# Wuziyi616/multi_part_assembly

Measured on AMD Instinct MI355X. Metric: train-step parts/sec (BxP) at N=1000 pts, higher is better.
Workload: dtype f32

## Files before the change

### multi_part_assembly_amd/csrc/coop_reduce.h

```cpp
#pragma once

#include <hip/hip_runtime.h>

namespace mpa {

template <int U, typename Load, typename Use>
__device__ __forceinline__ void batched_rows(int g, int G, int rows, Load load, Use use) {
  using T = decltype(load(0));
  int i = g;
  for (; i + (U - 1) * G < rows; i += U * G) {
    T t[U];
#pragma unroll
    for (int u = 0; u < U; ++u) t[u] = load(i + u * G);
#pragma unroll
    for (int u = 0; u < U; ++u) use(i + u * G, t[u]);
  }
  for (; i < rows; i += G) use(i, load(i));
}


constexpr int kSlices = 16;

constexpr int kEB = 64;

__device__ __forceinline__ void coop_store(double* p, double v) {
  __hip_atomic_store(reinterpret_cast<unsigned long long*>(p), (unsigned long long)__double_as_longlong(v), __ATOMIC_RELAXED,
                     __HIP_MEMORY_SCOPE_AGENT);
}
__device__ __forceinline__ double coop_load(const double* p) {
  return __longlong_as_double((long long)__hip_atomic_load(reinterpret_cast<const unsigned long long*>(p), __ATOMIC_RELAXED,
                                                           __HIP_MEMORY_SCOPE_AGENT));
}

struct CoopWs {
  double* stage;
  unsigned* ticket;
};

template <typename Row>
__device__ __forceinline__ bool coop_colsum(int total, int C, int c, const CoopWs ws, Row row, double& s0,
                                            double& s1) {
  __shared__ double sm[kSlices][64][2];
  __shared__ bool last;
  const int cl = threadIdx.x & 63, slice = threadIdx.x >> 6;
  const int g = blockIdx.y, G = gridDim.y;
  constexpr int U = kEB / kSlices;
  double x[U], y[U];
  bool ok[U];
#pragma unroll
  for (int u = 0; u < U; ++u) {
    const int e = g * kEB + slice + u * kSlices;
    row(e < total ? e : total - 1, ok[u], x[u], y[u]);
    ok[u] = ok[u] && e < total;
  }
  double a = 0.0, b = 0.0;
#pragma unroll
  for (int u = 0; u < U; ++u) {
    if (ok[u]) {
      a += x[u];
      b += y[u];
    }
  }
  sm[slice][cl][0] = a;
  sm[slice][cl][1] = b;
  __syncthreads();
  if (slice == 0) {
    a = b = 0.0;
#pragma unroll
    for (int k = 0; k < kSlices; ++k) {
      a += sm[k][cl][0];
      b += sm[k][cl][1];
    }
    coop_store(ws.stage + ((long long)g * C + c) * 2, a);
    coop_store(ws.stage + ((long long)g * C + c) * 2 + 1, b);
    asm volatile("s_waitcnt vmcnt(0)" ::: "memory");
  }
  __syncthreads();
  if (threadIdx.x == 0) last = atomicAdd(ws.ticket + blockIdx.x, 1u) == (unsigned)(G - 1);
  __syncthreads();
  if (!last) return false;
  a = b = 0.0;
  batched_rows<4>(slice, kSlices, G,
                  [&](int gg) {
                    const double* p = ws.stage + ((long long)gg * C + c) * 2;
                    return make_double2(coop_load(p), coop_load(p + 1));
                  },
                  [&](int, const double2 t) {
                    a += t.x;
                    b += t.y;
                  });
  sm[slice][cl][0] = a;
  sm[slice][cl][1] = b;
  __syncthreads();
  s0 = s1 = 0.0;
  if (slice == 0) {
#pragma unroll
    for (int k = 0; k < kSlices; ++k) {
      s0 += sm[k][cl][0];
      s1 += sm[k][cl][1];
    }
  }
  if (threadIdx.x == 0) ws.ticket[blockIdx.x] = 0u;
  return true;
}

}
```

### multi_part_assembly_amd/csrc/pn_bwd_q.h

```cpp

#ifdef PN_TIMING
#define PN_T_DECL unsigned long long t_busy = 0, t_mark = __builtin_amdgcn_s_memtime(), t_start = t_mark;
#define PN_BAR                                         \
  {                                                    \
    t_busy += __builtin_amdgcn_s_memtime() - t_mark;   \
    __syncthreads();                                   \
    t_mark = __builtin_amdgcn_s_memtime();             \
  }
#define PN_T_REPORT(ROLE)                                                                                              \
  if (blockIdx.x == 5 && lane == 0)                                                                                    \
    printf("K=%d FIRST=%d %s wave %d: units %d busy %llu of %llu cycles\n", K, (int)FIRST, ROLE, wave, n_it, t_busy, \
           __builtin_amdgcn_s_memtime() - t_start);
#else
#define PN_T_DECL
#define PN_BAR __syncthreads();
#define PN_T_REPORT(ROLE)
#endif
#define PN_LDS __attribute__((address_space(3)))
typedef short pn_s16x4 __attribute__((ext_vector_type(4)));
typedef short pn_s16x8 __attribute__((ext_vector_type(8)));
typedef unsigned int pn_u32x4 __attribute__((ext_vector_type(4)));

__device__ __forceinline__ pn_bf16x8 pn_tr_frag(const unsigned char* p, int stride) {
  const pn_s16x4 a = __builtin_amdgcn_ds_read_tr16_b64_v4i16((PN_LDS pn_s16x4*)p);
  const pn_s16x4 b = __builtin_amdgcn_ds_read_tr16_b64_v4i16((PN_LDS pn_s16x4*)(p + 4 * stride));
  const pn_s16x8 v = {a[0], a[1], a[2], a[3], b[0], b[1], b[2], b[3]};
  return __builtin_bit_cast(pn_bf16x8, v);
}

__device__ __forceinline__ void pn_split4(const float v[4], pn_bf16x4& ph, pn_bf16x4& pm, pn_bf16x4& pl) {
#pragma unroll
  for (int u = 0; u < 4; ++u) {
    ph[u] = (__bf16)v[u];
    const float r1 = v[u] - (float)ph[u];
    pm[u] = (__bf16)r1;
    pl[u] = (__bf16)(r1 - (float)pm[u]);
  }
}

typedef float pn_f32x2 __attribute__((ext_vector_type(2)));
typedef __bf16 pn_bf16x2 __attribute__((ext_vector_type(2)));
__device__ __forceinline__ void pn_split2v(pn_f32x2 x, pn_bf16x2& h, pn_bf16x2& m, pn_bf16x2& l) {
  h = __builtin_convertvector(x, pn_bf16x2);
  const pn_f32x2 r = x - __builtin_convertvector(h, pn_f32x2);
  m = __builtin_convertvector(r, pn_bf16x2);
  const pn_f32x2 t = r - __builtin_convertvector(m, pn_f32x2);
  l = __builtin_convertvector(t, pn_bf16x2);
}
__device__ __forceinline__ void pn_split4v(pn_f32x2 a, pn_f32x2 b, pn_bf16x4& ph, pn_bf16x4& pm, pn_bf16x4& pl) {
  pn_bf16x2 h0, m0, l0, h1, m1, l1;
  pn_split2v(a, h0, m0, l0);
  pn_split2v(b, h1, m1, l1);
  ph = pn_bf16x4{h0[0], h0[1], h1[0], h1[1]};
  pm = pn_bf16x4{m0[0], m0[1], m1[0], m1[1]};
  pl = pn_bf16x4{l0[0], l0[1], l1[0], l1[1]};
}

__device__ __forceinline__ void pn_fmac(float& acc, float a, float b) {
  asm volatile("v_fmac_f32 %0, %1, %2" : "+v"(acc) : "v"(a), "v"(b));
}

#define PN_MFMA6(ACC, AH, AM, AL, BH, BM, BL)                          \
  ACC = __builtin_amdgcn_mfma_f32_32x32x16_bf16(AH, BH, ACC, 0, 0, 0); \
  ACC = __builtin_amdgcn_mfma_f32_32x32x16_bf16(AH, BM, ACC, 0, 0, 0); \
  ACC = __builtin_amdgcn_mfma_f32_32x32x16_bf16(AM, BH, ACC, 0, 0, 0); \
  ACC = __builtin_amdgcn_mfma_f32_32x32x16_bf16(AM, BM, ACC, 0, 0, 0); \
  ACC = __builtin_amdgcn_mfma_f32_32x32x16_bf16(AH, BL, ACC, 0, 0, 0); \
  ACC = __builtin_amdgcn_mfma_f32_32x32x16_bf16(AL, BH, ACC, 0, 0, 0);

__global__ void pn_bwd_q_prep_kernel(const float* __restrict__ w, const float* __restrict__ coef, int K, int CIN,
                                     float* __restrict__ q) {
  const int k = blockIdx.x, d = threadIdx.x;
  float acc = 0.0f;
  if (k < CIN) {
#pragma unroll 8
    for (int c = 0; c < K; ++c) acc = __builtin_fmaf(coef[K + c] * w[(long long)c * CIN + k], w[(long long)c * CIN + d], acc);
  } else {
#pragma unroll 8
    for (int c = 0; c < K; ++c) acc = __builtin_fmaf(coef[2 * K + c], w[(long long)c * CIN + d], acc);
  }
  q[(long long)k * CIN + d] = acc;
}

__host__ __device__ constexpr int pn_bwd_q_elems(int K, int CIN, bool first) {
  return K * CIN + CIN * CIN + CIN + (first ? 192 + 12 : 0);
}

template <int N, typename F>
__device__ __forceinline__ void pn_static_for(F&& f) {
  if constexpr (N > 0) {
    pn_static_for<N - 1>(f);
    f(std::integral_constant<int, N - 1>{});
  }
}

struct PnWTile {
  signed char a, b, kind, orow, ocol;
};
template <int K>
struct PnWPlan;
template <>
struct PnWPlan<64> {
  static constexpr int TPW = 2;
  static constexpr PnWTile t[4][2] = {{{0, 8, 0, 0, 0}, {8, 8, 1, 0, 0}},
                                      {{0, 9, 0, 0, 1}, {8, 9, 1, 0, 1}},
                                      {{1, 8, 0, 1, 0}, {-1, -1, 0, 0, 0}},
                                      {{1, 9, 0, 1, 1}, {9, 9, 1, 1, 1}}};
  static constexpr int zc[4] = {0, 0, 1, 1};
  static constexpr bool uses(int w, int code) {
    for (int i = 0; i < TPW; ++i)
      if (t[w][i].a >= 0 && (t[w][i].a == code || t[w][i].b == code)) return true;
    return false;
  }
};
template <>
struct PnWPlan<128> {
  static constexpr int TPW = 3;
  static constexpr PnWTile t[4][3] = {{{0, 8, 0, 0, 0}, {0, 9, 0, 0, 1}, {8, 8, 1, 0, 0}},
                                      {{1, 8, 0, 1, 0}, {1, 9, 0, 1, 1}, {8, 9, 1, 0, 1}},
                                      {{2, 8, 0, 2, 0}, {2, 9, 0, 2, 1}, {9, 9, 1, 1, 1}},
                                      {{3, 8, 0, 3, 0}, {3, 9, 0, 3, 1}, {-1, -1, 0, 0, 0}}};
  static constexpr int zc[4] = {0, 1, 2, 3};
  static constexpr bool uses(int w, int code) {
    for (int i = 0; i < TPW; ++i)
      if (t[w][i].a >= 0 && (t[w][i].a == code || t[w][i].b == code)) return true;
    return false;
  }
};

template <int K, int CIN, int RB, int NS, int ND, int NW, bool FIRST, int KPN = 1>
__global__ __launch_bounds__(64 * (NS + ND + NW), (NS + ND + NW + 3) / 4) void pn_bwd_q_kernel(
    const float* __restrict__ dz, const float* __restrict__ y_prev, const float* __restrict__ bn_prev,
    const float* __restrict__ w, const float* __restrict__ coef, const float* __restrict__ q,
    const int* __restrict__ vlist, int N, float* __restrict__ dz_prev, float* __restrict__ partial,
    float* __restrict__ dwpart, const float* __restrict__ wt1) {
  constexpr int SZ = 6 * K + 16, SA = 6 * CIN + 16;
  constexpr int RT = RB / 32, CT = CIN / 32;
  constexpr int KZ = K / 16, KA = CIN / 16, KW = RB / 16;
  constexpr int NTS = 64 * NS, QK = K / 4, QC = CIN / 4, RG = NTS / QC;
  constexpr int NLZ = RB * QK / NTS, NLY = RB * QC / NTS;
  constexpr int ELEMS = pn_bwd_q_elems(K, CIN, FIRST);
  constexpr int OUTP = RB * CIN;
  static_assert(ND == RT * CT * KPN && RB * QK % NTS == 0 && RB * QC % NTS == 0 && NTS % QK == 0 && NTS % QC == 0, "shapes");
  static_assert(!FIRST || CIN == 64, "the recomputed input is the 64-channel first layer");
  __shared__ __attribute__((aligned(16))) unsigned char pz[2][RB * SZ];
  __shared__ __attribute__((aligned(16))) unsigned char pa[2][RB * SA];
  __shared__ __attribute__((aligned(16))) unsigned char wl[CIN * SZ];
  __shared__ __attribute__((aligned(16))) float outp[2][KPN][OUTP];
  const int wave = __builtin_amdgcn_readfirstlane(threadIdx.x >> 6), lane = threadIdx.x & 63, j = lane & 31, hh = lane >> 5;
  const int TB = (N + RB - 1) / RB, U = vlist[0] * TB, G = gridDim.x;
  const int n_it = (int)blockIdx.x < U ? (U - (int)blockIdx.x + G - 1) / G : 0;
  auto part_of = [&](int it) {
    const int u = (int)blockIdx.x + it * G;
    return u < U && it >= 0 ? vlist[4 + u / TB] : 0;
  };
  auto n0_of = [&](int it) { return (((int)blockIdx.x + it * G) % TB) * RB; };

  for (int e = threadIdx.x; e < CIN * (K / 4); e += blockDim.x) {
    const int d = e % CIN, k4 = e / CIN;
    float v[4];
#pragma unroll
    for (int u = 0; u < 4; ++u) v[u] = coef[4 * k4 + u] * w[(long long)(4 * k4 + u) * CIN + d];
    pn_bf16x4 ph, pm, pl;
    pn_split4(v, ph, pm, pl);
    unsigned char* p = wl + d * SZ + 8 * k4;
// ... 618 lines not shown
#pragma unroll
      for (int r = 0; r < 16; ++r) o[acc_row(r, hh) * CIN] = acc[r];
      PN_BAR
    }
    PN_T_REPORT("dgrad")
  } else {
    const int ww = wave - NS - ND;
    const int g16 = lane >> 4, i16 = lane & 15;
    const int trow = 8 * (g16 >> 1) + (i16 >> 2), tcol = 16 * (g16 & 1) + 4 * (i16 & 3);
    const int offa = trow * SA + 2 * tcol;
    constexpr int TPW = PnGPlan::TPW;
    f32x16 acc[TPW];
#pragma unroll
    for (int i = 0; i < TPW; ++i) acc[i] = f32x16{0};
    __syncthreads();
    PN_T_DECL
    auto run = [&](auto w_tag) {
      constexpr int W = decltype(w_tag)::value;
      for (int it = 0; it < n_it; ++it) {
        const unsigned char* ba = pa[it & 1] + offa;
        pn_bf16x8 f[4][3];
#pragma unroll
        for (int ks = 0; ks < KW; ++ks) {
          pn_static_for<4>([&](auto c_tag) {
            constexpr int c = decltype(c_tag)::value;
            if constexpr (PnGPlan::uses(W, c)) {
#pragma unroll
              for (int pl = 0; pl < 3; ++pl) f[c][pl] = pn_tr_frag(ba + 16 * ks * SA + 2 * CIN * pl + 64 * c, SA);
            }
          });
          pn_static_for<TPW>([&](auto i_tag) {
            constexpr int i = decltype(i_tag)::value;
            constexpr PnGTile tl = PnGPlan::t[W][i];
            if constexpr (tl.a >= 0) {
              PN_MFMA6(acc[i], f[tl.a][0], f[tl.a][1], f[tl.a][2], f[tl.b][0], f[tl.b][1], f[tl.b][2])
            }
          });
        }
        PN_BAR
      }
      float* out = dwpart + (long long)blockIdx.x * ELEMS;
      pn_static_for<TPW>([&](auto i_tag) {
        constexpr int i = decltype(i_tag)::value;
        constexpr PnGTile tl = PnGPlan::t[W][i];
        if constexpr (tl.a >= 0) {
#pragma unroll
          for (int r = 0; r < 16; ++r) {
            const int ra = 32 * tl.a + acc_row(r, hh), cb = 32 * tl.b + j;
            out[ra * CIN + cb] = acc[i][r];
            if (tl.a != tl.b) out[cb * CIN + ra] = acc[i][r];
          }
        }
      });
    };
    if (ww == 0) run(std::integral_constant<int, 0>{});
    else if (ww == 1) run(std::integral_constant<int, 1>{});
    else if (ww == 2) run(std::integral_constant<int, 2>{});
    else run(std::integral_constant<int, 3>{});
    PN_T_REPORT("gram")
  }
  __syncthreads();
  {
    const float* scr = reinterpret_cast<const float*>(&pa[0][0]);
    float* out = dwpart + (long long)blockIdx.x * ELEMS;
    const int t = threadIdx.x;
    if (t < 3 * CIN) {
      const int qq = t / CIN, c = t % CIN;
      float s = 0.0f;
#pragma unroll
      for (int g = 0; g < RG; ++g) s += scr[(qq * RG + g) * CIN + c];
      if (qq == 0) out[CIN * CIN + c] = s;
      else partial[((long long)blockIdx.x * CIN + c) * 2 + (qq - 1)] = s;
    }
  }
}

struct PnFinish {
  const float* red[3];
  const float* w[3];
  const float* coef[3];
  float* dw[3];
  int K[3], CIN[3], first[4];
  const float* w1;
  const float* coef1;
  float* dw1;
  int first_layer;
};
__global__ __launch_bounds__(256) void pn_bwd_finish_kernel(const PnFinish f) {
  if ((int)blockIdx.x == f.first[3]) {
    const int t = threadIdx.x;
    if (t >= 192) return;
    const int c = t / 3, k = t % 3, i = f.first_layer;
    const float* x = f.red[i] + f.K[i] * f.CIN[i] + f.CIN[i] * f.CIN[i] + f.CIN[i];
    const float* pp = x + 192;
    float wg = 0.0f;
#pragma unroll
    for (int jx = 0; jx < 3; ++jx) {
      const int a = jx < k ? jx : k, b = jx < k ? k : jx;
      wg = __builtin_fmaf(f.w1[c * 3 + jx], pp[a == 0 ? b : (a == 1 ? 2 + b : 5)], wg);
    }
    f.dw1[t] = f.coef1[c] * x[t] + f.coef1[64 + c] * wg + f.coef1[128 + c] * pp[6 + k];
    return;
  }
  int i = 0;
#pragma unroll
  for (int qq = 1; qq < 3; ++qq) i += (int)blockIdx.x >= f.first[qq] ? 1 : 0;
  const int K = f.K[i], CIN = f.CIN[i];
  const int e = ((int)blockIdx.x - f.first[i]) * 256 + threadIdx.x;
  if (e >= K * CIN) return;
  const int c = e / CIN, d = e % CIN;
  const float* T = f.red[i];
  const float* Gm = T + K * CIN;
  const float* asum = Gm + CIN * CIN;
  const float* wr = f.w[i] + (long long)c * CIN;
  float wg = 0.0f;
#pragma unroll 8
  for (int k = 0; k < CIN; ++k) {
    const float g = (k >> 5) <= (d >> 5) ? Gm[k * CIN + d] : Gm[d * CIN + k];
    wg = __builtin_fmaf(wr[k], g, wg);
  }
  f.dw[i][e] = f.coef[i][c] * T[e] + f.coef[i][K + c] * wg + f.coef[i][2 * K + c] * asum[d];
}
```

### multi_part_assembly_amd/csrc/pointnet.hip

```cpp
#include <type_traits>

#include "common.h"
#include "coop_reduce.h"

namespace {

constexpr int kT = 256;
using mpa::CoopWs;
using mpa::coop_colsum;
using mpa::kEB;
using mpa::kSlices;

typedef float f32x16 __attribute__((ext_vector_type(16)));

__device__ __forceinline__ int acc_row(int reg, int half) { return (reg & 3) + 8 * (reg >> 2) + 4 * half; }


__global__ __launch_bounds__(1024) void pn_count_kernel(const float* __restrict__ valids, int M, int N,
                                                        float* __restrict__ count, unsigned* __restrict__ ticket,
                                                        int* __restrict__ vlist, const float* __restrict__ w1 = nullptr,
                                                        float* __restrict__ wt1 = nullptr) {
  __shared__ int wcnt[16];
  if (threadIdx.x < 4) ticket[threadIdx.x] = 0u;
  if (w1 != nullptr && threadIdx.x < 192) wt1[(threadIdx.x % 3) * 64 + threadIdx.x / 3] = w1[threadIdx.x];
// ... 3 lines not shown
    const int m = m0 + threadIdx.x;
    const bool ok = m < M && valids[m] != 0.0f;
    const unsigned long long b = __ballot(ok);
    if (lane == 0) wcnt[wave] = __popcll(b);
    __syncthreads();
    int before = 0, total = 0;
#pragma unroll
    for (int k = 0; k < 16; ++k) {
      const int c = wcnt[k];
      before += k < wave ? c : 0;
      total += c;
    }
    if (ok) vlist[4 + base + before + __popcll(b & ((1ull << lane) - 1ull))] = m;
    base += total;
    __syncthreads();
  }
  if (threadIdx.x == 0) {
    count[0] = (float)base * (float)N;
    vlist[0] = base;
  }
}

__device__ __forceinline__ bool reduce_partials(const float* __restrict__ partial,
                                                const float* __restrict__ valids, int M, int splits, int C,
                                                int c, const CoopWs ws, double& s0, double& s1) {
  return coop_colsum(M * splits, C, c, ws,
                     [&](int e, bool& ok, double& x, double& y) {
                       const float2 v = *reinterpret_cast<const float2*>(partial + ((long long)e * C + c) * 2);
                       ok = valids == nullptr || valids[e / splits] != 0.0f;
                       x = (double)v.x;
                       y = (double)v.y;
                     },
                     s0, s1);
}

__global__ __launch_bounds__(64 * kSlices) void pn_bn_finalize_kernel(
    const float* __restrict__ partial, const float* __restrict__ valids, int M, int splits, int C,
    const float* __restrict__ count, const float* __restrict__ gamma, const float* __restrict__ beta,
    float* __restrict__ running_mean, float* __restrict__ running_var, float momentum, float eps,
    float* __restrict__ bn, const CoopWs cw) {
  const int c = blockIdx.x * 64 + (threadIdx.x & 63);
  double s, ss;
  if (!reduce_partials(partial, valids, M, splits, C, c, cw, s, ss)) return;
  if (threadIdx.x >= 64) return;
  const double n = (double)count[0];
  if (n == 0.0) {
    bn[c] = 0.0f;
    bn[C + c] = beta[c];
    bn[2 * C + c] = 0.0f;
    bn[3 * C + c] = 0.0f;
    return;
  }
  const double mean = s / n;
  double var = ss / n - mean * mean;
  if (var < 0.0) var = 0.0;
  const float invstd = (float)(1.0 / __builtin_sqrt(var + (double)eps));
  const float scale = gamma[c] * invstd;
  bn[c] = scale;
  bn[C + c] = beta[c] - (float)mean * scale;
  bn[2 * C + c] = (float)mean;
  bn[3 * C + c] = invstd;
  if (running_mean != nullptr) {
    const double unbiased = n > 1.0 ? var * n / (n - 1.0) : var;
    running_mean[c] = (1.0f - momentum) * running_mean[c] + momentum * (float)mean;
    running_var[c] = (1.0f - momentum) * running_var[c] + momentum * (float)unbiased;
  }
}

__global__ void pn_bn_from_running_kernel(int C, const float* __restrict__ gamma,
                                          const float* __restrict__ beta,
                                          const float* __restrict__ running_mean,
                                          const float* __restrict__ running_var, float eps,
                                          float* __restrict__ bn) {
  const int c = blockIdx.x * 64 + threadIdx.x;
  if (c >= C) return;
  const float invstd = 1.0f / __builtin_sqrtf(running_var[c] + eps);
  const float scale = gamma[c] * invstd;
  bn[c] = scale;
  bn[C + c] = beta[c] - running_mean[c] * scale;
  bn[2 * C + c] = running_mean[c];
  bn[3 * C + c] = invstd;
}

__device__ __forceinline__ void write_coef(float* __restrict__ coef, int C, int c, float gamma,
                                           const float* __restrict__ bn, double s1, double s2, double n) {
  const float mean = bn[2 * C + c], invstd = bn[3 * C + c];
  const float alpha = gamma * invstd;
  if (n == 0.0) {
    coef[c] = coef[C + c] = coef[2 * C + c] = 0.0f;
    return;
  }
  const float gammap = (float)(-(double)alpha * s2 / n * (double)invstd);
  coef[c] = alpha;
  coef[C + c] = gammap;
  coef[2 * C + c] = (float)(-(double)alpha * s1 / n - (double)gammap * (double)mean);
}

__global__ __launch_bounds__(64 * kSlices) void pn_bwd_coef_kernel(
    const float* __restrict__ partial, const float* __restrict__ valids, int M, int splits, int C,
    const float* __restrict__ count, const float* __restrict__ gamma, const float* __restrict__ bn,
    float* __restrict__ coef, float* __restrict__ dgamma, float* __restrict__ dbeta, const CoopWs cw) {
  const int c = blockIdx.x * 64 + (threadIdx.x & 63);
  double s1, s2;
  if (!reduce_partials(partial, valids, M, splits, C, c, cw, s1, s2)) return;
  if (threadIdx.x >= 64) return;
  write_coef(coef, C, c, gamma[c], bn, s1, s2, (double)count[0]);
  dgamma[c] = (float)s2;
  dbeta[c] = (float)s1;
}

__global__ __launch_bounds__(64 * kSlices) void pn_bwd_top_kernel(
    const float* __restrict__ gfeat, const int* __restrict__ argmax, const float* __restrict__ ybest,
    const float* __restrict__ valids, int M, int F, const float* __restrict__ count,
    const float* __restrict__ gamma, const float* __restrict__ bn, float* __restrict__ coef,
    float* __restrict__ dgamma, float* __restrict__ dbeta, const CoopWs cw) {
  const int c = blockIdx.x * 64 + (threadIdx.x & 63);
  const float mean = bn[2 * F + c], invstd = bn[3 * F + c];
  double s1, s2;
  const bool last = coop_colsum(M, F, c, cw,
                                [&](int m, bool& ok, double& x, double& y) {
                                  const long long o = (long long)m * F + c;
                                  const float g = gfeat[o];
                                  ok = valids[m] != 0.0f && argmax[o] >= 0;
                                  x = (double)g;
                                  y = (double)g * (double)((ybest[o] - mean) * invstd);
                                },
                                s1, s2);
  if (!last || threadIdx.x >= 64) return;
  write_coef(coef, F, c, gamma[c], bn, s1, s2, (double)count[0]);
  dgamma[c] = (float)s2;
  dbeta[c] = (float)s1;
}

struct Top2 {
  float v1, v2;
  int n1, n2;
};
constexpr int kNoIdx = 0x7fffffff;

__device__ __forceinline__ Top2 top2_empty() { return Top2{-__builtin_inff(), -__builtin_inff(), kNoIdx, kNoIdx}; }
__device__ __forceinline__ bool top2_before(float y, int n, float y2, int n2) {
  return y > y2 || (y == y2 && n < n2);
}
__device__ __forceinline__ void top2_push(Top2& t, float y, int n) {
  const bool g1 = y > t.v1, g2 = y > t.v2;
  t.v2 = g1 ? t.v1 : (g2 ? y : t.v2);
  t.n2 = g1 ? t.n1 : (g2 ? n : t.n2);
  t.v1 = g1 ? y : t.v1;
  t.n1 = g1 ? n : t.n1;
}
__device__ __forceinline__ Top2 top2_merge(const Top2 a, const Top2 b) {
  Top2 r;
  if (top2_before(b.v1, b.n1, a.v1, a.n1)) {
    r.v1 = b.v1;
    r.n1 = b.n1;
    const bool s = top2_before(a.v1, a.n1, b.v2, b.n2);
    r.v2 = s ? a.v1 : b.v2;
    r.n2 = s ? a.n1 : b.n2;
  } else {
    r.v1 = a.v1;
    r.n1 = a.n1;
    const bool s = top2_before(a.v2, a.n2, b.v1, b.n1);
    r.v2 = s ? a.v2 : b.v1;
    r.n2 = s ? a.n2 : b.n1;
  }
  return r;
}
__device__ __forceinline__ Top2 top2_shfl_xor(const Top2 t, int mask) {
  return Top2{__shfl_xor(t.v1, mask, 64), __shfl_xor(t.v2, mask, 64), __shfl_xor(t.n1, mask, 64),
              __shfl_xor(t.n2, mask, 64)};
}

__global__ void pn_top_finalize_kernel(const float* __restrict__ topv, const int* __restrict__ topn,
                                       const float* __restrict__ bn, const float* __restrict__ valids,
                                       const float* __restrict__ y4, const float* __restrict__ bn4,
                                       const float* __restrict__ w5, int M, int N, int F, int C4, int splits,
                                       float* __restrict__ feat, int* __restrict__ argmax,
                                       float* __restrict__ ybest) {
// ... 202 lines not shown
      float yv[UB];
#pragma unroll
      for (int u = 0; u < UB; ++u) {
        const int i = slice + (u0 + u) * S, arg = arg_s[i], mm = m0 + i < M ? m0 + i : M - 1;
        yv[u] = y4[((long long)mm * N + (arg >= 0 ? arg : 0)) * C4 + ci];
      }
      __builtin_amdgcn_sched_barrier(0);
#pragma unroll
      for (int u = 0; u < UB; ++u) {
        const int i = slice + (u0 + u) * S;
        if (arg_s[i] >= 0) acc = __builtin_fmaf(g_s[i], __builtin_fmaxf(__builtin_fmaf(yv[u], sc, sh), 0.0f), acc);
      }
    }
    __syncthreads();
  }
  float wg = 0.0f;
#pragma unroll
  for (int k = 0; k < C4 / S; ++k) wg = __builtin_fmaf(wk[k], gk[k], wg);
  sm[0][slice][ci] = acc;
  sm[1][slice][ci] = wg;
  __syncthreads();
  if (slice != 0) return;
  float sparse = 0.0f;
  wg = 0.0f;
#pragma unroll
  for (int k = 0; k < S; ++k) {
    sparse += sm[0][k][ci];
    wg += sm[1][k][ci];
  }
  dw5[(long long)c * C4 + ci] = coef[c] * sparse + coef[F + c] * wg + coef[2 * F + c] * gram[C4 * C4 + ci];
}

__device__ __forceinline__ float first_layer_y(float a0, float a1, float a2, float w0, float w1, float w2) {
  float v = a0 * w0;
  v = __builtin_fmaf(a1, w1, v);
  return __builtin_fmaf(a2, w2, v);
}

template <bool STORE>
__global__ __launch_bounds__(kT) void pn_fwd_first_kernel(const float* __restrict__ pts,
                                                          const float* __restrict__ wt,
                                                          const float* __restrict__ valids, int N,
                                                          float* __restrict__ y_out,
                                                          float* __restrict__ partial) {
  __shared__ float tile[kT / 64][64][65];
  __shared__ float red[kT / 64][64][2];
  const int m = blockIdx.y;
  if (valids[m] == 0.0f) return;
  const int wave = threadIdx.x >> 6, lane = threadIdx.x & 63;
  const int n0 = blockIdx.x * kT + wave * 64, n = n0 + lane;
  const long long row = (long long)m * N + (n < N ? n : N - 1);
  const int rows_here = N - n0 < 64 ? (N - n0 < 0 ? 0 : N - n0) : 64;
  const float a0 = pts[row * 3 + 0], a1 = pts[row * 3 + 1], a2 = pts[row * 3 + 2];
#pragma unroll
  for (int c = 0; c < 64; ++c) tile[wave][lane][c] = first_layer_y(a0, a1, a2, wt[c], wt[64 + c], wt[128 + c]);
  __builtin_amdgcn_wave_barrier();
  float s = 0.0f, ss = 0.0f;
  float* dst = y_out + ((long long)m * N + n0) * 64 + lane;
  for (int i = 0; i < rows_here; ++i) {
    const float v = tile[wave][i][lane];
    if constexpr (STORE) dst[(long long)i * 64] = v;
    s += v;
    ss = __builtin_fmaf(v, v, ss);
  }
  red[wave][lane][0] = s;
  red[wave][lane][1] = ss;
  __syncthreads();
  if (threadIdx.x < 64) {
    float t0 = 0.0f, t1 = 0.0f;
#pragma unroll
    for (int w = 0; w < kT / 64; ++w) {
      t0 += red[w][threadIdx.x][0];
      t1 += red[w][threadIdx.x][1];
    }
    const long long blk = (long long)m * gridDim.x + blockIdx.x;
    partial[(blk * 64 + threadIdx.x) * 2 + 0] = t0;
    partial[(blk * 64 + threadIdx.x) * 2 + 1] = t1;
  }
}

typedef __bf16 pn_bf16x8 __attribute__((ext_vector_type(8)));
typedef __bf16 pn_bf16x4 __attribute__((ext_vector_type(4)));

__global__ __launch_bounds__(64 * kSlices) void pn_wgrad_reduce_kernel(const float* __restrict__ dwpart,
                                                                      const float* __restrict__ valids,
                                                                      int M, int elems,
                                                                      float* __restrict__ dw) {
  __shared__ float sm[kSlices][64];
  const int el = threadIdx.x & 63, slice = threadIdx.x >> 6, i = blockIdx.x * 64 + el;
  float s = 0.0f;
  if (i < elems) {
    constexpr int U = 8;
    for (int m0 = slice; m0 < M; m0 += kSlices * U) {
      float v[U], ok[U];
#pragma unroll
      for (int u = 0; u < U; ++u) {
        const int m = m0 + u * kSlices, mm = m < M ? m : M - 1;
        v[u] = dwpart[(long long)mm * elems + i];
        ok[u] = m < M ? (valids != nullptr ? valids[mm] : 1.0f) : 0.0f;
      }
      __builtin_amdgcn_sched_barrier(0);
#pragma unroll
      for (int u = 0; u < U; ++u)
        if (ok[u] != 0.0f) s += v[u];
    }
  }
  sm[slice][el] = s;
  __syncthreads();
  if (slice == 0 && i < elems) {
    float t = 0.0f;
#pragma unroll
    for (int k = 0; k < kSlices; ++k) t += sm[k][el];
    dw[i] = t;
  }
}

struct WgradReduceGroup {
  const float* part[4];
  float* dw[4];
  int rows[4], elems[4], first[5];
};
__global__ __launch_bounds__(64 * kSlices) void pn_wgrad_reduce_group_kernel(const WgradReduceGroup g) {
  __shared__ float sm[kSlices][64];
  int k = 0;
#pragma unroll
  for (int q = 1; q < 4; ++q) k += (int)blockIdx.x >= g.first[q] ? 1 : 0;
  const float* __restrict__ dwpart = g.part[k];
  const int M = g.rows[k], elems = g.elems[k];
  const int el = threadIdx.x & 63, slice = threadIdx.x >> 6, i = ((int)blockIdx.x - g.first[k]) * 64 + el;
  float s = 0.0f;
  if (i < elems) {
    constexpr int U = 8;
    for (int m0 = slice; m0 < M; m0 += kSlices * U) {
      float v[U];
#pragma unroll
      for (int u = 0; u < U; ++u) {
        const int m = m0 + u * kSlices, mm = m < M ? m : M - 1;
        v[u] = dwpart[(long long)mm * elems + i];
      }
      __builtin_amdgcn_sched_barrier(0);
#pragma unroll
      for (int u = 0; u < U; ++u)
        if (m0 + u * kSlices < M) s += v[u];
    }
  }
  sm[slice][el] = s;
  __syncthreads();
  if (slice == 0 && i < elems) {
    float t = 0.0f;
#pragma unroll
    for (int q = 0; q < kSlices; ++q) t += sm[q][el];
    g.dw[k][i] = t;
  }
}

#include "pn_bwd_q.h"
#include "pn_fwd_ws.h"
#ifndef MPA_PN_FWD4_BLOCKS
#define MPA_PN_FWD4_BLOCKS 512
#endif
constexpr int kWsBlocks = 512;
static_assert(MPA_PN_FWD4_BLOCKS <= kWsBlocks, "every block of conv4's forward pass leaves one row of `partial`");

struct Dims {
  int64_t M, N, F, rows;
  int tiles1;
  int splits_top;
  int C[6];
};

Dims make_dims(int64_t M, int64_t N, int64_t F) {
  Dims d;
  d.M = M;
  d.N = N;
  d.F = F;
  d.rows = M * N;
  d.tiles1 = (int)((N + kT - 1) / kT);
  const int T = (int)((N + 31) / 32);
  d.splits_top = T >= 32 ? 8 : (T >= 16 ? 2 : 1);
  d.C[0] = 3;
  d.C[1] = 64;
  d.C[2] = 64;
  d.C[3] = 64;
  d.C[4] = 128;
  d.C[5] = (int)F;
  return d;
}

struct PnWs {
  float* Y[6];
  float* dZ[6];
  float* Wt1;
  float* bn[6];
  float* coef[6];
  float* partial;
  float* dwpart;
  float* count;
  CoopWs coop;
  float* topv;
  float* ybest;
  float* q;
  float* gram;
  float* ql[5];
  float* red[5];
  float* rsum;
  int64_t total;
};

struct PnIws {
  int* argmax;
  int* topn;
  int* vlist;
  int2* rtile;
  int64_t total;
};

PnWs carve(float* base, const Dims& d) {
  PnWs w;
  mpa::Arena a(base);
  w.Y[1] = nullptr;
  for (int l = 2; l <= 4; ++l) w.Y[l] = a.take<float>(d.rows * d.C[l], 16);
  w.Y[5] = nullptr;
  w.dZ[1] = nullptr;
  for (int l = 2; l <= 4; ++l) w.dZ[l] = a.take<float>(d.rows * d.C[l], 16);
  w.Wt1 = a.take<float>(192, 16);
  for (int l = 1; l <= 5; ++l) w.bn[l] = a.take<float>(4LL * d.C[l], 16);
  for (int l = 1; l <= 5; ++l) w.coef[l] = a.take<float>(4LL * d.C[l], 16);
  const int64_t maxc = d.F > 128 ? d.F : 128;
  int64_t blocks = d.M * (d.tiles1 > d.splits_top ? d.tiles1 : d.splits_top);
  if (blocks < kWsBlocks) blocks = kWsBlocks;
  w.partial = a.take<float>(blocks * maxc * 2, 16);
  {
    const int64_t gram = (int64_t)kWsBlocks * (128 * 128 + 128);
    const int64_t wait =
        (int64_t)kWsBlocks * (pn_bwd_q_elems(128, 64, false) + pn_bwd_q_elems(64, 64, false) + pn_bwd_q_elems(64, 64, true));
    w.dwpart = a.take<float>(gram > wait ? gram : wait, 16);
  }
  for (int l = 2; l <= 4; ++l) {
    w.ql[l] = a.take<float>((int64_t)(d.C[l - 1] + 1) * d.C[l - 1], 16);
    w.red[l] = a.take<float>(pn_bwd_q_elems(d.C[l], d.C[l - 1], l == 2), 16);
  }
  w.count = a.take<float>(4, 16);
  w.coop.ticket = a.take<unsigned>(4, 16);
  w.coop.stage = a.take<double>(2 * maxc * ((blocks + kEB - 1) / kEB), 16);
  w.topv = a.take<float>(d.M * d.splits_top * d.F * 2, 16);
  w.ybest = a.take<float>(d.M * d.F, 16);
  w.q = a.take<float>(129 * 128, 16);
  w.gram = a.take<float>(129 * 128, 16);
  w.rsum = a.take<float>(d.M * d.F * 128, 16);
  w.total = a.elems<float>();
  return w;
}

PnIws carve_int(int32_t* base, const Dims& d) {
  PnIws w;
  mpa::Arena a(base);
  w.argmax = a.take<int32_t>(d.M * d.F, 16);
  w.topn = a.take<int32_t>(d.M * d.splits_top * d.F * 2, 16);
  w.vlist = a.take<int32_t>(d.M + 4, 16);
  w.rtile = a.take<int2>(d.M * ((d.N + 31) / 32 + 1), 16);
  w.total = a.elems<int32_t>();
  return w;
}

int check_dims(int64_t M, int64_t N, int64_t F, const char* who) {
  MPA_REQUIRE(M >= 0 && N >= 1 && F >= 64, "%s: bad sizes", who);
  MPA_REQUIRE(F == 64 || F == 128 || F == 256, "%s: feat_dim must be 64, 128 or 256", who);
  MPA_REQUIRE(M <= 32767 && N <= 32768, "%s: at most 32767 parts of at most 32768 points", who);
  return MPA_OK;
}

}

extern "C" int mpa_pointnet_workspace(int64_t M, int64_t N, int64_t F, int64_t* float_elems,
                                      int64_t* int_elems) {
  if (int st = check_dims(M, N, F, "pointnet_workspace")) return st;
  MPA_REQUIRE(float_elems && int_elems, "pointnet_workspace: null pointer");
  const Dims d = make_dims(M, N, F);
  *float_elems = carve(nullptr, d).total;
  *int_elems = carve_int(nullptr, d).total;
  return MPA_OK;
}

extern "C" int mpa_pointnet_forward(const float* points, const float* valids, const float* const* conv_w,
                                    const float* const* bn_w, const float* const* bn_b,
                                    float* const* running_mean, float* const* running_var, int training,
                                    float momentum, float eps, int64_t M, int64_t N, int64_t F,
                                    float* float_ws, int32_t* int_ws, float* feat, void* stream) {
  if (int st = check_dims(M, N, F, "pointnet_forward")) return st;
  if (M == 0) return MPA_OK;
  MPA_REQUIRE(points && valids && conv_w && bn_w && bn_b && running_mean && running_var && float_ws &&
                  int_ws && feat, "pointnet_forward: null pointer");
  hipStream_t s = mpa::as_stream(stream);
  const Dims d = make_dims(M, N, F);
  const PnWs w = carve(float_ws, d);
  const PnIws iw = carve_int(int_ws, d);
  hipLaunchKernelGGL(pn_count_kernel, dim3(1), dim3(1024), 0, s, valids, (int)M, (int)N, w.count, w.coop.ticket,
                     iw.vlist, conv_w[0], w.Wt1);
  for (int l = 1; l <= 5; ++l) {
    int splits = 1;
    int prow_m = (int)M;
    const float* prow_valid = valids;
    if (l >= 2 && l <= 4) {
      prow_m = 256;
      prow_valid = nullptr;
      if (l == 2)
        hipLaunchKernelGGL((pn_fwd_ws_kernel<64, 64, 64, true>), dim3(256), dim3(768), 0, s, points, w.bn[1], conv_w[1], iw.vlist,
                           (int)N, w.Y[2], w.partial, (const float*)w.Wt1);
      else if (l == 3)
        hipLaunchKernelGGL((pn_fwd_ws_kernel<64, 64, 64, false>), dim3(256), dim3(768), 0, s, w.Y[2], w.bn[2], conv_w[2],
                           iw.vlist, (int)N, w.Y[3], w.partial, (const float*)nullptr);
      else {
        prow_m = MPA_PN_FWD4_BLOCKS;
        hipLaunchKernelGGL((pn_fwd_ws_kernel<64, 128, 32, false, 2>), dim3(MPA_PN_FWD4_BLOCKS), dim3(768), 0, s, w.Y[3], w.bn[3],
                           conv_w[3], iw.vlist, (int)N, w.Y[4], w.partial, (const float*)nullptr);
      }
    } else if (l == 1) {
      splits = d.tiles1;
      hipLaunchKernelGGL(pn_fwd_first_kernel<false>, dim3((unsigned)d.tiles1, (unsigned)M), dim3(kT), 0, s, points,
                         w.Wt1, valids, (int)N, (float*)nullptr, w.partial);
    } else {
      splits = d.splits_top;
#define MPA_FWD_TOP_WS(NWV)                                                                                               \
  hipLaunchKernelGGL((pn_fwd_ws_top_kernel<128, NWV>), dim3(256), dim3(64 * (4 + NWV)), 0, s, w.Y[4], w.bn[4], conv_w[4],  \
                     d.C[5], iw.vlist, (int)N, splits, w.partial, w.topv, iw.topn, bn_w[4])
      if (F == 256) MPA_FWD_TOP_WS(8);
      else if (F == 128) MPA_FWD_TOP_WS(4);
      else MPA_FWD_TOP_WS(2);
#undef MPA_FWD_TOP_WS
    }
    const dim3 cg((unsigned)(d.C[l] / 64));
    if (training)
      hipLaunchKernelGGL(pn_bn_finalize_kernel, dim3(cg.x, (unsigned)(((long long)prow_m * splits + kEB - 1) / kEB)),
                         dim3(64 * kSlices), 0, s, w.partial, prow_valid, prow_m, splits, d.C[l], w.count, bn_w[l - 1],
                         bn_b[l - 1], running_mean[l - 1], running_var[l - 1], momentum, eps, w.bn[l], w.coop);
    else
      hipLaunchKernelGGL(pn_bn_from_running_kernel, cg, dim3(64), 0, s, d.C[l], bn_w[l - 1], bn_b[l - 1],
                         running_mean[l - 1], running_var[l - 1], eps, w.bn[l]);
  }
  hipLaunchKernelGGL(pn_top_finalize_kernel, dim3((unsigned)((M * F + 255) / 256)), dim3(256), 0, s, w.topv, iw.topn,
                     w.bn[5], valids, w.Y[4], w.bn[4], conv_w[4], (int)M, (int)N, (int)F, d.C[4], d.splits_top, feat,
                     iw.argmax, w.ybest);
  return mpa::check_launch("pointnet_forward");
}

extern "C" int mpa_pointnet_backward(const float* grad_feat, const float* points, const float* valids,
                                     const float* const* conv_w, const float* const* bn_w, int64_t M,
                                     int64_t N, int64_t F, float* float_ws, const int32_t* int_ws,
                                     float* const* grad_conv_w, float* const* grad_bn_w,
                                     float* const* grad_bn_b, void* stream) {
  if (int st = check_dims(M, N, F, "pointnet_backward")) return st;
  if (M == 0) return MPA_OK;
  MPA_REQUIRE(grad_feat && points && valids && conv_w && bn_w && float_ws && int_ws && grad_conv_w &&
                  grad_bn_w && grad_bn_b, "pointnet_backward: null pointer");
  hipStream_t s = mpa::as_stream(stream);
  const Dims d = make_dims(M, N, F);
  const PnWs w = carve(float_ws, d);
  const PnIws iw = carve_int(const_cast<int32_t*>(int_ws), d);
  const int C4 = d.C[4];
  hipLaunchKernelGGL(pn_bwd_top_kernel, dim3((unsigned)(F / 64), (unsigned)((M + kEB - 1) / kEB)), dim3(64 * kSlices),
                     0, s, grad_feat, iw.argmax, w.ybest, valids, (int)M, (int)F, w.count, bn_w[4], w.bn[5],
                     w.coef[5], grad_bn_w[4], grad_bn_b[4], w.coop);
  hipLaunchKernelGGL(pn_top_csr_kernel, dim3((unsigned)(M + C4 + 1)), dim3(kTopRowsThreads),
                     sizeof(int) * pn_top_csr_lds_words((int)F, (int)((N + 31) / 32)), s, iw.argmax, grad_feat, w.coef[5], valids, (int)N,
                     (int)F, iw.rtile, w.rsum, (int)M, conv_w[4], w.q);
  hipLaunchKernelGGL((pn_bwd_top_q_kernel<128, 4, 4, 4>), dim3(256), dim3(768), 0, s, w.Y[4], w.bn[4], w.q, iw.vlist, (int)N,
                     w.dZ[4], w.partial, w.dwpart, iw.rtile, w.rsum, (int)F);
  hipLaunchKernelGGL(pn_bwd_coef_kernel, dim3((unsigned)(C4 / 64), (unsigned)((256 + kEB - 1) / kEB)), dim3(64 * kSlices), 0, s,
                     w.partial, (const float*)nullptr, 256, 1, C4, w.count, bn_w[3], w.bn[4], w.coef[4], grad_bn_w[3],
                     grad_bn_b[3], w.coop);
  hipLaunchKernelGGL(pn_wgrad_reduce_kernel, dim3((unsigned)((C4 * C4 + C4 + 63) / 64)), dim3(64 * kSlices), 0, s, w.dwpart,
                     (const float*)nullptr, 256, C4 * C4 + C4, w.gram);
  hipLaunchKernelGGL(pn_top_wgrad_kernel, dim3((unsigned)F), dim3(1024), 0, s, grad_feat, iw.argmax, valids, w.Y[4],
                     w.bn[4], conv_w[4], w.coef[5], w.gram, (int)M, (int)N, (int)F, grad_conv_w[4]);
  WgradReduceGroup rg{};
  PnFinish fin{};
  long long part_off = 0;
  for (int l = 4, i = 0; l >= 2; --l, ++i) {
    const int cout = d.C[l], cin = d.C[l - 1], elems = pn_bwd_q_elems(cout, cin, l == 2);
    hipLaunchKernelGGL(pn_bwd_q_prep_kernel, dim3((unsigned)(cin + 1)), dim3((unsigned)cin), 0, s, conv_w[l - 1], w.coef[l],
                       cout, cin, w.ql[l]);
    float* const dwl = w.dwpart + part_off;
#define MPA_QK(KK, RBB, NSS, NDD, NWW, FI, YP)                                                                        \
  hipLaunchKernelGGL((pn_bwd_q_kernel<KK, 64, RBB, NSS, NDD, NWW, FI, (KK == 128 ? 2 : 1)>), dim3(nb),                  \
                     dim3(64 * (NSS + NDD + NWW)), 0,                                                                   \
                     s, w.dZ[l], YP, w.bn[l - 1], conv_w[l - 1], w.coef[l], w.ql[l], iw.vlist, (int)N, w.dZ[l - 1],    \
                     w.partial, dwl, (const float*)w.Wt1)
    const int nb = 256;
    if (l == 2) MPA_QK(64, 64, 4, 4, 4, true, points);
    else if (cout == 64) MPA_QK(64, 64, 4, 4, 4, false, w.Y[l - 1]);
    else MPA_QK(128, 32, 4, 4, 4, false, w.Y[l - 1]);
#undef MPA_QK
    hipLaunchKernelGGL(pn_bwd_coef_kernel, dim3((unsigned)(cin / 64), (unsigned)((nb + kEB - 1) / kEB)),
                       dim3(64 * kSlices), 0, s, w.partial, (const float*)nullptr, nb, 1, cin, w.count, bn_w[l - 2],
                       w.bn[l - 1], w.coef[l - 1], grad_bn_w[l - 2], grad_bn_b[l - 2], w.coop);
    rg.part[i] = dwl;
    rg.dw[i] = w.red[l];
    rg.rows[i] = nb;
    rg.elems[i] = elems;
    fin.red[i] = w.red[l];
    fin.w[i] = conv_w[l - 1];
    fin.coef[i] = w.coef[l];
    fin.dw[i] = grad_conv_w[l - 1];
    fin.K[i] = cout;
    fin.CIN[i] = cin;
    part_off += (long long)nb * elems;
  }
  rg.first[0] = 0;
  fin.first[0] = 0;
  for (int k = 0; k < 4; ++k) rg.first[k + 1] = rg.first[k] + (k < 3 ? (rg.elems[k] + 63) / 64 : 0);
  for (int k = 0; k < 3; ++k) fin.first[k + 1] = fin.first[k] + (fin.K[k] * fin.CIN[k] + 255) / 256;
  fin.w1 = conv_w[0];
  fin.coef1 = w.coef[1];
  fin.dw1 = grad_conv_w[0];
  fin.first_layer = 2;
  hipLaunchKernelGGL(pn_wgrad_reduce_group_kernel, dim3((unsigned)rg.first[4]), dim3(64 * kSlices), 0, s, rg);
  hipLaunchKernelGGL(pn_bwd_finish_kernel, dim3((unsigned)(fin.first[3] + 1)), dim3(256), 0, s, fin);
  return mpa::check_launch("pointnet_backward");
}
```

Measured before the change: 383,800.

## Fold top gram reduction and first-layer BN coef into grouped backward kernels

The top layer's dwpart reduction moves out of its own kernel and into the grouped wgrad reduce as a fourth table, and pn_top_wgrad is deferred until after that grouped launch. The last layer's BN coefficient kernel is dropped; the finish kernel's first-layer block now column-sums the partials itself (block_colsum), computes the coefficients and BN grads, and uses them directly. This cuts two kernel launches and their serialization on the stream. In exchange, a single block does the 256x128 reduction serially, and the workspace layout is reshuffled under a static_assert.

```diff
diff --git a/multi_part_assembly_amd/csrc/coop_reduce.h b/multi_part_assembly_amd/csrc/coop_reduce.h
--- a/multi_part_assembly_amd/csrc/coop_reduce.h
+++ b/multi_part_assembly_amd/csrc/coop_reduce.h
@@ -104,4 +104,49 @@
   return true;
 }
 
+__host__ __device__ constexpr int block_colsum_groups(int rows) { return (rows + kEB - 1) / kEB; }
+template <int KB>
+__device__ __forceinline__ void block_colsum(const float* __restrict__ table, int rows, int C, double* groups,
+                                             double* tot) {
+  static_assert(kSlices % KB == 0, "slices per batch");
+  constexpr int U = kEB / kSlices;
+  const int G = block_colsum_groups(rows), C2 = 2 * C;
+  const auto rsrc = __builtin_amdgcn_make_buffer_rsrc(const_cast<float*>(table), 0, rows * C2 * 4, 0x00020000);
+  for (int item = threadIdx.x; item < G * C2; item += blockDim.x) {
+    const int g = item / C2, cq = item % C2;
+    const int voff = (g * kEB * C2 + cq) * 4;
+    double gs = 0.0;
+#pragma unroll 1
+    for (int k0 = 0; k0 < kSlices; k0 += KB) {
+      float v[KB][U];
+#pragma unroll
+      for (int k = 0; k < KB; ++k)
+#pragma unroll
+        for (int u = 0; u < U; ++u)
+          v[k][u] = __builtin_bit_cast(float, __builtin_amdgcn_raw_buffer_load_b32(rsrc, voff, (k0 + k + u * kSlices) * C2 * 4, 0));
+#pragma unroll
+      for (int k = 0; k < KB; ++k) {
+        double a = 0.0;
+#pragma unroll
+        for (int u = 0; u < U; ++u)
+          if (g * kEB + k0 + k + u * kSlices < rows) a += (double)v[k][u];
+        gs += a;
+      }
+    }
+    groups[item] = gs;
+  }
+  __syncthreads();
+  for (int cq = threadIdx.x; cq < C2; cq += blockDim.x) {
+    double t = 0.0;
+#pragma unroll 1
+    for (int s = 0; s < kSlices; ++s) {
+      double a = 0.0;
+      for (int gg = s; gg < G; gg += kSlices) a += groups[gg * C2 + cq];
+      t += a;
+    }
+    tot[cq] = t;
+  }
+  __syncthreads();
 }
+
+}
diff --git a/multi_part_assembly_amd/csrc/pn_bwd_q.h b/multi_part_assembly_amd/csrc/pn_bwd_q.h
--- a/multi_part_assembly_amd/csrc/pn_bwd_q.h
+++ b/multi_part_assembly_amd/csrc/pn_bwd_q.h
@@ -81,6 +81,8 @@
   }
   q[(long long)k * CIN + d] = acc;
 }
+
+constexpr int kBwdBlocks = 256;
 
 __host__ __device__ constexpr int pn_bwd_q_elems(int K, int CIN, bool first) {
   return K * CIN + CIN * CIN + CIN + (first ? 192 + 12 : 0);
@@ -865,13 +867,34 @@
   float* dw[3];
   int K[3], CIN[3], first[4];
   const float* w1;
-  const float* coef1;
+  float* coef1;
   float* dw1;
   int first_layer;
+  const float* partial1;
+  const float* count;
+  const float* gamma1;
+  const float* bn1;
+  float* dgamma1;
+  float* dbeta1;
 };
 __global__ __launch_bounds__(256) void pn_bwd_finish_kernel(const PnFinish f) {
+  __shared__ double groups1[mpa::block_colsum_groups(kBwdBlocks) * 64 * 2];
+  __shared__ double tot1[64 * 2];
+  __shared__ float coef1_s[3][64];
   if ((int)blockIdx.x == f.first[3]) {
     const int t = threadIdx.x;
+    mpa::block_colsum<16>(f.partial1, kBwdBlocks, 64, groups1, tot1);
+    if (t < 64) {
+      const double s1 = tot1[2 * t], s2 = tot1[2 * t + 1];
+      float alpha, gammap, betap;
+      coef_values(f.gamma1[t], f.bn1[2 * 64 + t], f.bn1[3 * 64 + t], s1, s2, (double)f.count[0], alpha, gammap, betap);
+      coef1_s[0][t] = f.coef1[t] = alpha;
+      coef1_s[1][t] = f.coef1[64 + t] = gammap;
+      coef1_s[2][t] = f.coef1[128 + t] = betap;
+      f.dgamma1[t] = (float)s2;
+      f.dbeta1[t] = (float)s1;
+    }
+    __syncthreads();
     if (t >= 192) return;
     const int c = t / 3, k = t % 3, i = f.first_layer;
     const float* x = f.red[i] + f.K[i] * f.CIN[i] + f.CIN[i] * f.CIN[i] + f.CIN[i];
@@ -882,7 +905,7 @@
       const int a = jx < k ? jx : k, b = jx < k ? k : jx;
       wg = __builtin_fmaf(f.w1[c * 3 + jx], pp[a == 0 ? b : (a == 1 ? 2 + b : 5)], wg);
     }
-    f.dw1[t] = f.coef1[c] * x[t] + f.coef1[64 + c] * wg + f.coef1[128 + c] * pp[6 + k];
+    f.dw1[t] = coef1_s[0][c] * x[t] + coef1_s[1][c] * wg + coef1_s[2][c] * pp[6 + k];
     return;
   }
   int i = 0;
diff --git a/multi_part_assembly_amd/csrc/pointnet.hip b/multi_part_assembly_amd/csrc/pointnet.hip
--- a/multi_part_assembly_amd/csrc/pointnet.hip
+++ b/multi_part_assembly_amd/csrc/pointnet.hip
@@ -109,18 +109,24 @@
   bn[3 * C + c] = invstd;
 }
 
+__device__ __forceinline__ void coef_values(float gamma, float mean, float invstd, double s1, double s2, double n,
+                                            float& alpha, float& gammap, float& betap) {
+  alpha = gamma * invstd;
+  if (n == 0.0) {
+    alpha = gammap = betap = 0.0f;
+    return;
+  }
+  gammap = (float)(-(double)alpha * s2 / n * (double)invstd);
+  betap = (float)(-(double)alpha * s1 / n - (double)gammap * (double)mean);
+}
+
 __device__ __forceinline__ void write_coef(float* __restrict__ coef, int C, int c, float gamma,
                                            const float* __restrict__ bn, double s1, double s2, double n) {
-  const float mean = bn[2 * C + c], invstd = bn[3 * C + c];
-  const float alpha = gamma * invstd;
-  if (n == 0.0) {
-    coef[c] = coef[C + c] = coef[2 * C + c] = 0.0f;
-    return;
-  }
-  const float gammap = (float)(-(double)alpha * s2 / n * (double)invstd);
+  float alpha, gammap, betap;
+  coef_values(gamma, bn[2 * C + c], bn[3 * C + c], s1, s2, n, alpha, gammap, betap);
   coef[c] = alpha;
   coef[C + c] = gammap;
-  coef[2 * C + c] = (float)(-(double)alpha * s1 / n - (double)gammap * (double)mean);
+  coef[2 * C + c] = betap;
 }
 
 __global__ __launch_bounds__(64 * kSlices) void pn_bwd_coef_kernel(
@@ -489,39 +495,6 @@
 typedef __bf16 pn_bf16x8 __attribute__((ext_vector_type(8)));
 typedef __bf16 pn_bf16x4 __attribute__((ext_vector_type(4)));
 
-__global__ __launch_bounds__(64 * kSlices) void pn_wgrad_reduce_kernel(const float* __restrict__ dwpart,
-                                                                      const float* __restrict__ valids,
-                                                                      int M, int elems,
-                                                                      float* __restrict__ dw) {
-  __shared__ float sm[kSlices][64];
-  const int el = threadIdx.x & 63, slice = threadIdx.x >> 6, i = blockIdx.x * 64 + el;
-  float s = 0.0f;
-  if (i < elems) {
-    constexpr int U = 8;
-    for (int m0 = slice; m0 < M; m0 += kSlices * U) {
-      float v[U], ok[U];
-#pragma unroll
-      for (int u = 0; u < U; ++u) {
-        const int m = m0 + u * kSlices, mm = m < M ? m : M - 1;
-        v[u] = dwpart[(long long)mm * elems + i];
-        ok[u] = m < M ? (valids != nullptr ? valids[mm] : 1.0f) : 0.0f;
-      }
-      __builtin_amdgcn_sched_barrier(0);
-#pragma unroll
-      for (int u = 0; u < U; ++u)
-        if (ok[u] != 0.0f) s += v[u];
-    }
-  }
-  sm[slice][el] = s;
-  __syncthreads();
-  if (slice == 0 && i < elems) {
-    float t = 0.0f;
-#pragma unroll
-    for (int k = 0; k < kSlices; ++k) t += sm[k][el];
-    dw[i] = t;
-  }
-}
-
 struct WgradReduceGroup {
   const float* part[4];
   float* dw[4];
@@ -638,10 +611,10 @@
   if (blocks < kWsBlocks) blocks = kWsBlocks;
   w.partial = a.take<float>(blocks * maxc * 2, 16);
   {
-    const int64_t gram = (int64_t)kWsBlocks * (128 * 128 + 128);
-    const int64_t wait =
-        (int64_t)kWsBlocks * (pn_bwd_q_elems(128, 64, false) + pn_bwd_q_elems(64, 64, false) + pn_bwd_q_elems(64, 64, true));
-    w.dwpart = a.take<float>(gram > wait ? gram : wait, 16);
+    constexpr int64_t gram = 128 * 128 + 128;
+    constexpr int64_t wait = pn_bwd_q_elems(128, 64, false) + pn_bwd_q_elems(64, 64, false) + pn_bwd_q_elems(64, 64, true);
+    static_assert(kBwdBlocks * (gram + wait) <= kWsBlocks * wait, "the four tables fit");
+    w.dwpart = a.take<float>(kWsBlocks * (gram > wait ? gram : wait), 16);
   }
   for (int l = 2; l <= 4; ++l) {
     w.ql[l] = a.take<float>((int64_t)(d.C[l - 1] + 1) * d.C[l - 1], 16);
@@ -776,13 +749,10 @@
   hipLaunchKernelGGL(pn_bwd_coef_kernel, dim3((unsigned)(C4 / 64), (unsigned)((256 + kEB - 1) / kEB)), dim3(64 * kSlices), 0, s,
                      w.partial, (const float*)nullptr, 256, 1, C4, w.count, bn_w[3], w.bn[4], w.coef[4], grad_bn_w[3],
                      grad_bn_b[3], w.coop);
-  hipLaunchKernelGGL(pn_wgrad_reduce_kernel, dim3((unsigned)((C4 * C4 + C4 + 63) / 64)), dim3(64 * kSlices), 0, s, w.dwpart,
-                     (const float*)nullptr, 256, C4 * C4 + C4, w.gram);
-  hipLaunchKernelGGL(pn_top_wgrad_kernel, dim3((unsigned)F), dim3(1024), 0, s, grad_feat, iw.argmax, valids, w.Y[4],
-                     w.bn[4], conv_w[4], w.coef[5], w.gram, (int)M, (int)N, (int)F, grad_conv_w[4]);
   WgradReduceGroup rg{};
   PnFinish fin{};
-  long long part_off = 0;
+  const int nb = kBwdBlocks;
+  long long part_off = (long long)nb * (C4 * C4 + C4);
   for (int l = 4, i = 0; l >= 2; --l, ++i) {
     const int cout = d.C[l], cin = d.C[l - 1], elems = pn_bwd_q_elems(cout, cin, l == 2);
     hipLaunchKernelGGL(pn_bwd_q_prep_kernel, dim3((unsigned)(cin + 1)), dim3((unsigned)cin), 0, s, conv_w[l - 1], w.coef[l],
@@ -793,14 +763,14 @@
                      dim3(64 * (NSS + NDD + NWW)), 0,                                                                   \
                      s, w.dZ[l], YP, w.bn[l - 1], conv_w[l - 1], w.coef[l], w.ql[l], iw.vlist, (int)N, w.dZ[l - 1],    \
                      w.partial, dwl, (const float*)w.Wt1)
-    const int nb = 256;
     if (l == 2) MPA_QK(64, 64, 4, 4, 4, true, points);
     else if (cout == 64) MPA_QK(64, 64, 4, 4, 4, false, w.Y[l - 1]);
     else MPA_QK(128, 32, 4, 4, 4, false, w.Y[l - 1]);
 #undef MPA_QK
-    hipLaunchKernelGGL(pn_bwd_coef_kernel, dim3((unsigned)(cin / 64), (unsigned)((nb + kEB - 1) / kEB)),
-                       dim3(64 * kSlices), 0, s, w.partial, (const float*)nullptr, nb, 1, cin, w.count, bn_w[l - 2],
-                       w.bn[l - 1], w.coef[l - 1], grad_bn_w[l - 2], grad_bn_b[l - 2], w.coop);
+    if (l > 2)
+      hipLaunchKernelGGL(pn_bwd_coef_kernel, dim3((unsigned)(cin / 64), (unsigned)((nb + kEB - 1) / kEB)),
+                         dim3(64 * kSlices), 0, s, w.partial, (const float*)nullptr, nb, 1, cin, w.count, bn_w[l - 2],
+                         w.bn[l - 1], w.coef[l - 1], grad_bn_w[l - 2], grad_bn_b[l - 2], w.coop);
     rg.part[i] = dwl;
     rg.dw[i] = w.red[l];
     rg.rows[i] = nb;
@@ -813,15 +783,27 @@
     fin.CIN[i] = cin;
     part_off += (long long)nb * elems;
   }
+  rg.part[3] = w.dwpart;
+  rg.dw[3] = w.gram;
+  rg.rows[3] = nb;
+  rg.elems[3] = C4 * C4 + C4;
   rg.first[0] = 0;
   fin.first[0] = 0;
-  for (int k = 0; k < 4; ++k) rg.first[k + 1] = rg.first[k] + (k < 3 ? (rg.elems[k] + 63) / 64 : 0);
+  for (int k = 0; k < 4; ++k) rg.first[k + 1] = rg.first[k] + (rg.elems[k] + 63) / 64;
   for (int k = 0; k < 3; ++k) fin.first[k + 1] = fin.first[k] + (fin.K[k] * fin.CIN[k] + 255) / 256;
   fin.w1 = conv_w[0];
   fin.coef1 = w.coef[1];
   fin.dw1 = grad_conv_w[0];
   fin.first_layer = 2;
+  fin.partial1 = w.partial;
+  fin.count = w.count;
+  fin.gamma1 = bn_w[0];
+  fin.bn1 = w.bn[1];
+  fin.dgamma1 = grad_bn_w[0];
+  fin.dbeta1 = grad_bn_b[0];
   hipLaunchKernelGGL(pn_wgrad_reduce_group_kernel, dim3((unsigned)rg.first[4]), dim3(64 * kSlices), 0, s, rg);
+  hipLaunchKernelGGL(pn_top_wgrad_kernel, dim3((unsigned)F), dim3(1024), 0, s, grad_feat, iw.argmax, valids, w.Y[4],
+                     w.bn[4], conv_w[4], w.coef[5], w.gram, (int)M, (int)N, (int)F, grad_conv_w[4]);
   hipLaunchKernelGGL(pn_bwd_finish_kernel, dim3((unsigned)(fin.first[3] + 1)), dim3(256), 0, s, fin);
   return mpa::check_launch("pointnet_backward");
 }
```

Measured after the change: 380,200, median of 2. Within noise of the previous version (-0.9%).
